# aoschu/esn-ofdm-mimo

Hardware: AMD Instinct MI355X
Metric: OFDM symbols/s through the ESN detector (4x8 TDL-B, N=128, N_res=512; train+predict+detect) (higher is better)
Workload: dtype f16 operands / f32 accumulate

## Files before the change

### esn_ofdm_mimo_amd/csrc/esn_solve.hip

```cpp
#include <stdlib.h>
#include <type_traits>
#include "esn_common.h"
#include "esn_launch.h"

namespace esn {

struct SolveParams {
    const double* E; const double* D;
    const float* E32;
    int n_groups, T, transient, cols, n_out;
    const double* t_scale; const double* t_shift;
    double* W_out; int* status;
    double* work; size_t work_stride;
    int m, n, wide;
    int skip;
    int part_ok;
    int vec;
    int dma;
    unsigned long long* stamps;
    const double* ridge; int n_ridge;
};

__device__ __forceinline__ bool ridge_rejects(const SolveParams& sp, int slot) {
    const double lam = sp.ridge[slot];
// ... 128 lines not shown
            double* z = R + (size_t)o * m;
            for (int j = 0; j < n; ++j) {
                const double* cj = M + (size_t)j * m;
                double acc = 0.0;
                for (int k = lane; k < j; k += 64) acc = fma(cj[k], z[k], acc);
                acc = wave_sum(acc);
                if (lane == 0) {
                    double d = rdiag[j];
                    z[j] = (fabs(d) > tol) ? (z[j] - acc) / d : 0.0;
                }
                __builtin_amdgcn_s_waitcnt(0);
                __builtin_amdgcn_wave_barrier();
            }
            for (int j = n - 1; j >= 0; --j) {
                const double* cj = M + (size_t)j * m;
                const double b = beta[j];
                if (b == 0.0) continue;
                double dot = 0.0;
                for (int i = j + lane; i < m; i += 64) dot = fma(cj[i], z[i], dot);
                dot = wave_sum(dot) * b;
                for (int i = j + lane; i < m; i += 64) z[i] = fma(-dot, cj[i], z[i]);
                __builtin_amdgcn_s_waitcnt(0);
                __builtin_amdgcn_wave_barrier();
            }
            double* wo = sp.W_out + ((size_t)slot * nrhs + o) * cols;
            for (int i = lane; i < cols; i += 64) wo[i] = z[i];
        }
    } else {
        for (int o = wv; o < nrhs; o += nwv) {
            double* c = M + (size_t)(n + o) * m;
            for (int j = n - 1; j >= 0; --j) {
                double acc = 0.0;
                for (int k = j + 1 + lane; k < n; k += 64) acc = fma(M[(size_t)k * m + j], c[k], acc);
                acc = wave_sum(acc);
                if (lane == 0) {
                    double d = rdiag[j];
                    c[j] = (fabs(d) > tol) ? (c[j] - acc) / d : 0.0;
                }
                __builtin_amdgcn_s_waitcnt(0);
                __builtin_amdgcn_wave_barrier();
            }
            double* wo = sp.W_out + ((size_t)slot * nrhs + o) * cols;
            for (int i = lane; i < n; i += 64) wo[i] = c[i];
        }
    }
}

size_t solve_work_doubles(int rows, int cols, int n_out) {
    const bool wide = rows < cols;
    const size_t m = wide ? cols : rows, n = wide ? rows : cols;
    size_t d = (n + (wide ? 0 : n_out)) * m + (size_t)n_out * m + 2 * n;
    return (d + 1) & ~(size_t)1;
}

size_t solve_ridge_work_doubles(int rows, int cols, int n_out) {
    const bool wide = rows < cols;
    const size_t m = (size_t)rows + cols, n = wide ? rows : cols;
    size_t d = (n + (wide ? 0 : n_out)) * m + (size_t)n_out * m + 2 * n;
    return (d + 1) & ~(size_t)1;
}

int launch_readout_solve(const double* E, const double* D, int n_groups, int T, int transient,
                         int cols, int n_out, const double* t_scale, const double* t_shift,
                         double* W_out, int* status, void* workspace, hipStream_t stream,
                         const double* ridge, int n_ridge) {
    SolveParams sp;
    const int rows = T - transient;
    sp.ridge = ridge; sp.n_ridge = n_ridge;
    sp.E = E; sp.E32 = nullptr; sp.D = D; sp.n_groups = n_groups; sp.T = T; sp.transient = transient;
    sp.cols = cols; sp.n_out = n_out; sp.t_scale = t_scale; sp.t_shift = t_shift;
    sp.W_out = W_out; sp.status = status;
    sp.work = reinterpret_cast<double*>(workspace);
    sp.work_stride = ridge ? solve_ridge_work_doubles(rows, cols, n_out) : solve_work_doubles(rows, cols, n_out);
    sp.wide = rows < cols;
    sp.m = sp.wide ? cols : rows;
    sp.n = sp.wide ? rows : cols;
    if (ridge) hipLaunchKernelGGL(readout_qr_kernel<true>, dim3(n_groups * n_ridge), dim3(1024), 0, stream, sp);
    else hipLaunchKernelGGL(readout_qr_kernel<false>, dim3(n_groups), dim3(1024), 0, stream, sp);
    return (int)hipGetLastError();
}

}

namespace esn {

constexpr int CH_NP = 128;
constexpr int CH_NT = 512;
constexpr int CH_NW = CH_NT / 64;
constexpr int CH_TILES = 36;
constexpr int CH_KC = 32;
constexpr int CH_AS_LD = CH_NP + 16;
constexpr int CH_RHS = 8;
constexpr size_t CH_LDS = sizeof(double) * ((size_t)CH_TILES * 256 + (size_t)CH_NP * CH_RHS);
static_assert(2 * CH_KC * CH_AS_LD <= CH_TILES * 256, "E staging aliases the Gram tiles");

typedef double f64x4 __attribute__((ext_vector_type(4)));

constexpr int CH_RING = 4;
constexpr int CH_RBUF = CH_KC * CH_NP * 4;
constexpr int CH_WRING = 3;
constexpr int CH_WSEG = 8192;
constexpr int CH_WROWS = 4;
static_assert(CH_RING * CH_RBUF <= CH_TILES * 256 * 8, "Gram ring aliases the Gram tiles");
static_assert(CH_WRING * 3 * CH_WSEG <= CH_TILES * 256 * 8, "W_out ring aliases the Gram tiles");

__device__ __forceinline__ __amdgpu_buffer_rsrc_t ch_rsrc(const void* ptr, int bytes) {
    const uint64_t a = (uint64_t)reinterpret_cast<uintptr_t>(ptr);
    const uint32_t lo = __builtin_amdgcn_readfirstlane((uint32_t)a);
    const uint32_t hi = __builtin_amdgcn_readfirstlane((uint32_t)(a >> 32));
    return __builtin_amdgcn_make_buffer_rsrc(reinterpret_cast<char*>((uintptr_t)(((uint64_t)hi << 32) | lo)), 0,
                                             __builtin_amdgcn_readfirstlane(bytes), 0x00020000);
}
__device__ __forceinline__ void ch_dma16(__amdgpu_buffer_rsrc_t rs, char* dst, int voff) {
    __builtin_amdgcn_raw_ptr_buffer_load_lds(rs, (__attribute__((address_space(3))) void*)dst, 16, voff, 0, 0, 0);
}
constexpr int CH_OOR = 0x7ffffff0;
__device__ __forceinline__ void ch_wait_dma(int pending) {
    switch (pending) {
        case 4: asm volatile("s_waitcnt vmcnt(4) lgkmcnt(0)" ::: "memory"); break;
        case 3: asm volatile("s_waitcnt vmcnt(3) lgkmcnt(0)" ::: "memory"); break;
        case 2: asm volatile("s_waitcnt vmcnt(2) lgkmcnt(0)" ::: "memory"); break;
        default: asm volatile("s_waitcnt vmcnt(0) lgkmcnt(0)" ::: "memory"); break;
    }
}

__device__ __forceinline__ void ch_wrow(const char* e, const double* al, float (&a)[4], double (&b)[8]) {
    typedef float f32x4 __attribute__((ext_vector_type(4)));
    typedef double f64x2 __attribute__((ext_vector_type(2)));
    const uint32_t ea = (uint32_t)(uintptr_t)(const __attribute__((address_space(3))) char*)e;
    const uint32_t ba = (uint32_t)(uintptr_t)(const __attribute__((address_space(3))) double*)al;
    f32x4 ev;
    f64x2 b0, b1, b2, b3;
    asm volatile("ds_read_b128 %0, %5\n\tds_read_b128 %1, %6\n\tds_read_b128 %2, %6 offset:16\n\t"
                 "ds_read_b128 %3, %6 offset:32\n\tds_read_b128 %4, %6 offset:48\n\ts_waitcnt lgkmcnt(0)"
                 : "=v"(ev), "=v"(b0), "=v"(b1), "=v"(b2), "=v"(b3) : "v"(ea), "v"(ba) : "memory");
    a[0] = ev.x; a[1] = ev.y; a[2] = ev.z; a[3] = ev.w;
    b[0] = b0.x; b[1] = b0.y; b[2] = b1.x; b[3] = b1.y; b[4] = b2.x; b[5] = b2.y; b[6] = b3.x; b[7] = b3.y;
}

__device__ __forceinline__ int ch_tile(int ti, int tj) { return (ti * (ti + 1) / 2 + tj) * 256; }
__device__ __forceinline__ int ch_el(int r, int c) { return r * 16 + (c ^ (r & ~1)); }

__device__ __forceinline__ void ch_load4(const float* p, float (&v)[4]) {
    const float4 x = *reinterpret_cast<const float4*>(p);
    v[0] = x.x; v[1] = x.y; v[2] = x.z; v[3] = x.w;
}
__device__ __forceinline__ void ch_load4(const double* p, double (&v)[4]) {
    const double2 x = *reinterpret_cast<const double2*>(p), y = *reinterpret_cast<const double2*>(p + 2);
    v[0] = x.x; v[1] = x.y; v[2] = y.x; v[3] = y.y;
}
__device__ __forceinline__ const float* ch_src(const SolveParams& sp, float*) { return sp.E32; }
__device__ __forceinline__ const double* ch_src(const SolveParams& sp, double*) { return sp.E; }

__device__ __forceinline__ double ch_bcast(double x, int src) {
    const uint64_t u = __builtin_bit_cast(uint64_t, x);
    const uint32_t lo = __builtin_amdgcn_readlane((uint32_t)u, src);
    const uint32_t hi = __builtin_amdgcn_readlane((uint32_t)(u >> 32), src);
    return __builtin_bit_cast(double, ((uint64_t)hi << 32) | lo);
}

__device__ __forceinline__ int ch_factor_diag(double* D, int j0, int n, double piv_tol, int lane) {
    const int r = lane & 15;
    double a[16], x[16];
#pragma unroll
    for (int c = 0; c < 16; ++c) a[c] = D[ch_el(r, c)];
    double my_invd = 1.0;
    unsigned rejected = 0, dropped = 0;
#pragma unroll
    for (int j = 0; j < 16; ++j) {
        const double v = ch_bcast(a[j], j);
        const bool live = j0 + j < n;
        const bool ok = live && v > piv_tol;
        if (live && !ok) rejected |= 1u << j;
        if (!ok) dropped |= 1u << j;
        const double d = ok ? sqrt(v) : 1.0, inv_d = ok ? 1.0 / d : 0.0;
        if (r == j) my_invd = ok ? inv_d : 1.0;
        a[j] = (r == j) ? d : ((r > j) ? a[j] * inv_d : 0.0);
#pragma unroll
        for (int k = j + 1; k < 16; ++k) {
            const double lkj = ch_bcast(a[j], k);
            if (r >= k) a[k] = fma(-a[j], lkj, a[k]);
        }
    }
#pragma unroll
    for (int i = 0; i < 16; ++i) {
        double sacc = (i == r) ? 1.0 : 0.0;
#pragma unroll
        for (int k = 0; k < i; ++k) sacc = fma(-ch_bcast(a[k], i), x[k], sacc);
        const double idi = ch_bcast(my_invd, i);
        x[i] = (i >= r && !((dropped >> i) & 1u)) ? sacc * idi : 0.0;
    }
    if (lane < 16) {
#pragma unroll
        for (int i = 0; i < 16; ++i) D[ch_el(i, r)] = x[i];
    }
    return rejected ? 1 : 0;
}

template <typename TE, bool wide, bool RG>
__global__ __launch_bounds__(CH_NT) __attribute__((amdgpu_waves_per_eu(4))) void readout_chol_kernel(SolveParams sp) {
    extern __shared__ __attribute__((aligned(16))) char chol_smem[];
    double* Gs = reinterpret_cast<double*>(chol_smem);
    double* As = Gs;
    double* Bs = Gs + CH_TILES * 256;
    const int slot = blockIdx.x, tid = threadIdx.x;
    const int g = RG ? slot / sp.n_ridge : slot;
    if constexpr (RG) {
        if (ridge_rejects(sp, slot)) return;
    }
    const int lane = tid & 63, wv = __builtin_amdgcn_readfirstlane(tid >> 6);
    const int lr = lane & 15, lq = lane >> 4;
    const int rows = sp.T - sp.transient, cols = sp.cols, nrhs = sp.n_out;
    const int n = wide ? rows : cols;
    const int m = wide ? cols : rows;
    const int ntile = (n + 15) / 16;
    const TE* A = ch_src(sp, (TE*)nullptr) + ((size_t)g * sp.T + sp.transient) * cols;
    const double* Dg = sp.D + ((size_t)g * sp.T + sp.transient) * nrhs;

    int g_ti[5], g_tj[5];
    const int g_cnt = wv < 4 ? 5 : 4;
#pragma unroll
    for (int q = 0; q < 5; ++q) {
        const int t = wv + CH_NW * q < CH_TILES ? wv + CH_NW * q : 0;
        int ti = 0;
        while ((ti + 1) * (ti + 2) / 2 <= t) ++ti;
        g_ti[q] = ti;
        g_tj[q] = t - ti * (ti + 1) / 2;
    }
    f64x4 acc[5];
#pragma unroll
    for (int q = 0; q < 5; ++q) acc[q] = f64x4{0.0, 0.0, 0.0, 0.0};
    double atb[2] = {0.0, 0.0};
    auto run_of = [&](int p, int& i, int& kk) {
        const int e = tid + CH_NT * p;
        if (wide) { i = (e & 15) + 16 * ((e >> 7) & 7); kk = 4 * ((e >> 4) & 7); }
        else      { kk = e >> 5; i = 4 * (e & 31); }
    };
    TE stg[2][4];
    auto fetch = [&](int k0) {
#pragma unroll
        for (int p = 0; p < 2; ++p) {
            int i, kk;
            run_of(p, i, kk);
            const int k = k0 + kk;
            int nv = wide ? (i < n ? m - k : 0) : (k < m ? n - i : 0);
            nv = nv < 0 ? 0 : (nv > 4 ? 4 : nv);
            const TE* src = A + (wide ? (size_t)i * cols + k : (size_t)k * cols + i);
            if (nv == 4 && sp.vec) {
                ch_load4(src, stg[p]);
            } else {
#pragma unroll
                for (int j = 0; j < 4; ++j) stg[p][j] = j < nv ? src[j] : (TE)0;
            }
        }
    };
    auto commit = [&](double* dst) {
#pragma unroll
        for (int p = 0; p < 2; ++p) {
            int i, kk;
            run_of(p, i, kk);
#pragma unroll
            for (int j = 0; j < 4; ++j) {
                if (wide) dst[(kk + j) * CH_AS_LD + i] = (double)stg[p][j];
                else      dst[kk * CH_AS_LD + i + j] = (double)stg[p][j];
            }
        }
    };
    double* Abuf[2] = {As, As + CH_KC * CH_AS_LD};
    const int m_run = (sp.skip & 1) ? CH_KC : m;
    constexpr bool can_dma = wide && sizeof(TE) == 4;
    const bool dma = can_dma && sp.dma && sp.vec;
#ifdef ESN_STAMPS
    unsigned long long st_acc[8] = {0, 0, 0, 0, 0, 0, 0, 0}, st_ph[4] = {0, 0, 0, 0};
    ESN_STAMP(st_k0);
#endif
    if constexpr (can_dma) {
        if (dma) {
            char* ring = chol_smem;
            const __amdgpu_buffer_rsrc_t ers = ch_rsrc(A, n * cols * 4);
            const int kq = lane >> 3;
            int roff[2];
#pragma unroll
            for (int j = 0; j < 2; ++j) roff[j] = ((16 * wv + 8 * j + (lane & 7)) * cols + 4 * kq) * 4;
            const int nch = (m_run + CH_KC - 1) / CH_KC;
            auto issue = [&](int c, int b) {
                const int k0 = c * CH_KC;
                const bool ok = k0 + 4 * kq < m;
#pragma unroll
                for (int j = 0; j < 2; ++j)
                    ch_dma16(ers, ring + b * CH_RBUF + (2 * wv + j) * 1024, ok ? roff[j] + 4 * k0 : CH_OOR);
            };
#pragma unroll
            for (int c = 0; c < CH_RING - 1; ++c)
                if (c < nch) issue(c, c);
            const int lbase = 1024 * (lr >> 3) + 16 * (lr & 7) + 4 * lq;
            for (int c = 0, b = 0; c < nch; ++c, b = (b + 1 == CH_RING ? 0 : b + 1)) {
#ifdef ESN_STAMPS
                ESN_STAMP(s0);
#endif
                const int later = nch - 1 - c < CH_RING - 2 ? nch - 1 - c : CH_RING - 2;
                ch_wait_dma(2 * later);
#ifdef ESN_STAMPS
                ESN_STAMP(s1);
#endif
                __builtin_amdgcn_s_barrier();
                if (c + CH_RING - 1 < nch) issue(c + CH_RING - 1, b == 0 ? CH_RING - 1 : b - 1);
                const char* buf = ring + b * CH_RBUF + lbase;
                const float* pa[5];
                const float* pb[5];
#pragma unroll
                for (int q = 0; q < 5; ++q) {
                    pa[q] = reinterpret_cast<const float*>(buf + 2048 * g_ti[q]);
                    pb[q] = reinterpret_cast<const float*>(buf + 2048 * g_tj[q]);
                }
#ifdef ESN_STAMPS
                ESN_STAMP(s2);
                {
                    float x = pa[0][0];
                    asm volatile("" :: "v"(x));
                }
                ESN_STAMP(s3);
#endif
                auto step = [&](int s, auto cnt) {
#pragma unroll
                    for (int q = 0; q < decltype(cnt)::value; ++q)
                        acc[q] = __builtin_amdgcn_mfma_f64_16x16x4f64((double)pa[q][32 * s], (double)pb[q][32 * s], acc[q], 0, 0, 0);
                };
                const int kmax = (m - c * CH_KC < CH_KC) ? m - c * CH_KC : CH_KC;
                if (kmax == CH_KC && g_cnt == 5) {
#pragma unroll
                    for (int s = 0; s < CH_KC / 4; ++s) step(s, std::integral_constant<int, 5>());
                } else if (kmax == CH_KC) {
#pragma unroll
                    for (int s = 0; s < CH_KC / 4; ++s) step(s, std::integral_constant<int, 4>());
                } else if (g_cnt == 5) {
                    for (int s = 0; s < kmax / 4; ++s) step(s, std::integral_constant<int, 5>());
                } else {
                    for (int s = 0; s < kmax / 4; ++s) step(s, std::integral_constant<int, 4>());
                }
#ifdef ESN_STAMPS
                ESN_STAMP(s4);
                st_acc[0] += s1 - s0; st_acc[1] += s2 - s1; st_acc[2] += s3 - s2; st_acc[3] += s4 - s3;
#endif
            }
            __syncthreads();
        }
    }
    for (int k0 = 0, cur = 0; k0 < (dma ? 0 : m_run); k0 += CH_KC, cur ^= 1) {
        if (k0 == 0) {
            fetch(0);
            commit(Abuf[0]);
            __syncthreads();
        }
#ifdef ESN_STAMPS
        ESN_STAMP(s0);
#endif
        if (k0 + CH_KC < m_run) fetch(k0 + CH_KC);
        const double* Ac = Abuf[cur];
        const int kmax = (m - k0 < CH_KC) ? m - k0 : CH_KC;
        const double* slab0 = Ac + lq * CH_AS_LD + lr;
        for (int k4 = 0; k4 < kmax; k4 += 4) {
            const double* slab = slab0 + k4 * CH_AS_LD;
#pragma unroll
            for (int q = 0; q < 5; ++q)
                if (q < g_cnt)
                    acc[q] = __builtin_amdgcn_mfma_f64_16x16x4f64(slab[g_ti[q] * 16], slab[g_tj[q] * 16], acc[q], 0, 0, 0);
        }
        if constexpr (!wide) {
#pragma unroll
            for (int p = 0; p < 2; ++p) {
                const int e = tid + CH_NT * p, o = e / CH_NP, i = e % CH_NP;
                if (o < nrhs) {
                    const double sc = sp.t_scale ? sp.t_scale[(size_t)g * nrhs + o] : 1.0;
                    const double sh = sp.t_shift ? sp.t_shift[(size_t)g * nrhs + o] : 0.0;
                    for (int kk = 0; kk < kmax; ++kk)
                        atb[p] = fma(Ac[kk * CH_AS_LD + i], Dg[(size_t)(k0 + kk) * nrhs + o] * sc + sh, atb[p]);
                }
            }
        }
#ifdef ESN_STAMPS
        ESN_STAMP(s1);
#endif
        if (k0 + CH_KC < m_run) commit(Abuf[cur ^ 1]);
#ifdef ESN_STAMPS
        ESN_STAMP(s2);
#endif
        __syncthreads();
#ifdef ESN_STAMPS
        ESN_STAMP(s3);
        st_acc[3] += s1 - s0; st_acc[0] += s2 - s1; st_acc[1] += s3 - s2;
#endif
    }
#ifdef ESN_STAMPS
    ESN_STAMP(st_k1);
#endif

#pragma unroll
    for (int q = 0; q < 5; ++q)
        if (q < g_cnt) {
            double* T = Gs + ch_tile(g_ti[q], g_tj[q]);
#pragma unroll
            for (int i = 0; i < 4; ++i) T[ch_el(4 * i + lq, lr)] = acc[q][i];
        }
#pragma unroll
    for (int p = 0; p < 2; ++p) {
        const int e = tid + CH_NT * p;
        if (wide) {
            const int i = e / CH_RHS, o = e % CH_RHS;
            double v = 0.0;
            if (i < n && o < nrhs) {
                const double sc = sp.t_scale ? sp.t_scale[(size_t)g * nrhs + o] : 1.0;
                const double sh = sp.t_shift ? sp.t_shift[(size_t)g * nrhs + o] : 0.0;
                v = Dg[(size_t)i * nrhs + o] * sc + sh;
            }
            Bs[e] = v;
        } else {
            const int o = e / CH_NP, i = e % CH_NP;
            Bs[i * CH_RHS + o] = (o < nrhs && i < n) ? atb[p] : 0.0;
        }
    }
    __syncthreads();
    if constexpr (RG) {
        const double lam = sp.ridge[slot];
        for (int i = tid; i < n; i += CH_NT) Gs[ch_tile(i >> 4, i >> 4) + ch_el(i & 15, i & 15)] += lam;
        __syncthreads();
    }

    int bad = 0;
    const int nblk = (sp.skip & 2) ? 1 : ntile;
    double piv_tol = 0.0;
    if (wv == 0) {
        double dmax = 0.0;
        for (int i = lane; i < n; i += 64) dmax = fmax(dmax, Gs[ch_tile(i >> 4, i >> 4) + ch_el(i & 15, i & 15)]);
#pragma unroll
        for (int off = 32; off > 0; off >>= 1) dmax = fmax(dmax, __shfl_xor(dmax, off));
        piv_tol = dmax * 1e-14;
    }
    for (int kb = -1; kb < nblk; ++kb) {
        if (kb >= 0) {
            const int rt = kb + 1 + wv;
            if (rt < ntile) {
                const double* Li = Gs + ch_tile(kb, kb);

                double* T = Gs + ch_tile(rt, kb);
                f64x4 c = {0.0, 0.0, 0.0, 0.0};
#pragma unroll
                for (int k0 = 0; k0 < 16; k0 += 4)
                    c = __builtin_amdgcn_mfma_f64_16x16x4f64(T[ch_el(lr, k0 + lq)], Li[ch_el(lr, k0 + lq)], c, 0, 0, 0);
#pragma unroll
                for (int i = 0; i < 4; ++i) T[ch_el(4 * i + lq, lr)] = c[i];
            }
        }
        if (kb >= 0) {
            __syncthreads();
            const int mt = ntile - kb - 1, cnt = mt * (mt + 1) / 2;
            for (int t = wv; t < cnt; t += (wv == 0 ? cnt : CH_NW - 1)) {
                int di = 0;
                while ((di + 1) * (di + 2) / 2 <= t) ++di;
                const int ti = kb + 1 + di, tj = kb + 1 + t - di * (di + 1) / 2;
                double* C = Gs + ch_tile(ti, tj);
                const double* La = Gs + ch_tile(ti, kb);
                const double* Lb = Gs + ch_tile(tj, kb);
                f64x4 c;
#pragma unroll
                for (int i = 0; i < 4; ++i) c[i] = C[ch_el(4 * i + lq, lr)];
#pragma unroll
                for (int k0 = 0; k0 < 16; k0 += 4)
                    c = __builtin_amdgcn_mfma_f64_16x16x4f64(-La[ch_el(lr, k0 + lq)], Lb[ch_el(lr, k0 + lq)], c, 0, 0, 0);
#pragma unroll
                for (int i = 0; i < 4; ++i) C[ch_el(4 * i + lq, lr)] = c[i];
            }
        }
        if (wv == 0 && kb + 1 < nblk) bad |= ch_factor_diag(Gs + ch_tile(kb + 1, kb + 1), 16 * (kb + 1), n, piv_tol, lane);
        __syncthreads();
    }

#ifdef ESN_STAMPS
    ESN_STAMP(st_k2);
#endif
    if (!(sp.skip & 4)) {
        const bool bl = lr < CH_RHS;
        f64x4 keep = {0.0, 0.0, 0.0, 0.0};
        int keep_t = -1;
        auto rhs_tile = [&](int I) -> f64x4 {
            f64x4 v;
#pragma unroll
            for (int i = 0; i < 4; ++i) v[i] = bl ? Bs[(16 * I + 4 * i + lq) * CH_RHS + lr] : 0.0;
            return v;
        };
        auto put_tile = [&](int I, const f64x4& v) {
            if (bl) {
#pragma unroll
                for (int i = 0; i < 4; ++i) Bs[(16 * I + 4 * i + lq) * CH_RHS + lr] = v[i];
            }
        };
        auto flush = [&]() {
            if (wv == CH_NW - 1 && keep_t >= 0) put_tile(keep_t, keep);
            keep_t = -1;
        };
        for (int I = 0; I < ntile; ++I) {
            flush();
            const int J = I + 1 + wv;
            const bool upd = J < ntile;
            if (upd || wv == CH_NW - 1) {
                const double* Li = Gs + ch_tile(I, I);
                const f64x4 b = rhs_tile(I);
                f64x4 z = {0.0, 0.0, 0.0, 0.0};
#pragma unroll
                for (int s = 0; s < 4; ++s)
                    z = __builtin_amdgcn_mfma_f64_16x16x4f64(Li[ch_el(lr, 4 * s + lq)], b[s], z, 0, 0, 0);
                if (upd) {
                    const double* L = Gs + ch_tile(J, I);
                    f64x4 c = rhs_tile(J);
#pragma unroll
                    for (int s = 0; s < 4; ++s)
                        c = __builtin_amdgcn_mfma_f64_16x16x4f64(-L[ch_el(lr, 4 * s + lq)], z[s], c, 0, 0, 0);
                    put_tile(J, c);
                } else {
                    keep = z;
                    keep_t = I;
                }
            }
            __syncthreads();
        }
        flush();
        __syncthreads();
        for (int I = ntile - 1; I >= 0; --I) {
            flush();
            const int J = wv;
            const bool upd = J < I;
            if (upd || wv == CH_NW - 1) {
                const double* Li = Gs + ch_tile(I, I);
                const f64x4 zi = rhs_tile(I);
                f64x4 x = {0.0, 0.0, 0.0, 0.0};
#pragma unroll
                for (int s = 0; s < 4; ++s)
                    x = __builtin_amdgcn_mfma_f64_16x16x4f64(Li[ch_el(4 * s + lq, lr)], zi[s], x, 0, 0, 0);
                if (upd) {
                    const double* L = Gs + ch_tile(I, J);
                    f64x4 c = rhs_tile(J);
#pragma unroll
                    for (int s = 0; s < 4; ++s)
                        c = __builtin_amdgcn_mfma_f64_16x16x4f64(-L[ch_el(4 * s + lq, lr)], x[s], c, 0, 0, 0);
                    put_tile(J, c);
                } else {
                    keep = x;
                    keep_t = I;
                }
            }
            __syncthreads();
        }
        flush();
        __syncthreads();
    }

#ifdef ESN_STAMPS
    ESN_STAMP(st_k3);
#endif
    if constexpr (wide) {
        constexpr int CPT = 16 / sizeof(TE);
        const int nunit = cols / CPT;
        int parts = nunit > 0 ? CH_NT / nunit : 0;
        parts = parts > 3 ? 3 : parts;
        if (sp.vec && cols % CPT == 0 && parts > 0 && (parts - 1) * CH_RHS * cols <= CH_TILES * 256 && !(sp.skip & 8)) {
            double* part = Gs;
            const int pt = tid / nunit, un = tid - pt * nunit;
            double w[CPT][CH_RHS];
#pragma unroll
            for (int c = 0; c < CPT; ++c)
#pragma unroll
                for (int o = 0; o < CH_RHS; ++o) w[c][o] = 0.0;
            const int per = (n + parts - 1) / parts;
            int rw = CH_WSEG / (cols * 4);
            rw = rw > CH_WROWS ? CH_WROWS : rw;
            bool wdma = false;
            if constexpr (can_dma) {
              wdma = dma && rw > 0;
              if (wdma) {
                char* ring = chol_smem;
                const __amdgpu_buffer_rsrc_t ers = ch_rsrc(A, n * cols * 4);
                const int rowb = cols * 4;
                const int nch = (per + rw - 1) / rw;
                auto issue = [&](int c, int b) {
#pragma unroll
                    for (int j = 0; j < 3; ++j) {
                        const int r0 = j * per + c * rw;
                        int nr = (j < parts) ? ((j + 1) * per < n ? (j + 1) * per : n) - r0 : 0;
                        nr = nr < 0 ? 0 : (nr > rw ? rw : nr);
                        const int off = 1024 * wv + 16 * lane;
                        ch_dma16(ers, ring + (b * 3 + j) * CH_WSEG + 1024 * wv, off < nr * rowb ? r0 * rowb + off : CH_OOR);
                    }
                };
#pragma unroll
                for (int c = 0; c < CH_WRING - 1; ++c)
                    if (c < nch) issue(c, c);
                const int i0 = pt * per, i1 = (i0 + per < n) ? i0 + per : n;
                for (int c = 0, b = 0; c < nch; ++c, b = (b + 1 == CH_WRING ? 0 : b + 1)) {
#ifdef ESN_STAMPS
                    ESN_STAMP(s0);
#endif
                    ch_wait_dma(nch - 1 - c < CH_WRING - 2 ? 3 * (nch - 1 - c) : 3 * (CH_WRING - 2));
#ifdef ESN_STAMPS
                    ESN_STAMP(s1);
#endif
                    __builtin_amdgcn_s_barrier();
                    if (c + CH_WRING - 1 < nch) issue(c + CH_WRING - 1, b == 0 ? CH_WRING - 1 : b - 1);
#ifdef ESN_STAMPS
                    ESN_STAMP(s2);
#endif
                    if (pt < parts) {
                        const char* seg = ring + (b * 3 + pt) * CH_WSEG + CPT * sizeof(TE) * un;
                        const int ib = i0 + c * rw;
                        const int nr = ((ib + rw < i1) ? ib + rw : i1) - ib;
#pragma unroll
                        for (int rr = 0; rr < CH_WROWS; ++rr) {
                            if (rr >= nr) break;
                            const int i = ib + rr;
                            float a[4];
                            double al[CH_RHS];
                            ch_wrow(seg + rr * rowb, Bs + i * CH_RHS, a, al);
#pragma unroll
                            for (int o = 0; o < CH_RHS; ++o)
                                if (o < nrhs) {
#pragma unroll
                                    for (int cc = 0; cc < CPT; ++cc) w[cc][o] = fma((double)a[cc], al[o], w[cc][o]);
                                }
                        }
                    }
#ifdef ESN_STAMPS
                    ESN_STAMP(s3);
                    st_acc[4] += s1 - s0; st_acc[5] += s2 - s1; st_acc[6] += s3 - s2;
#endif
                }
                __syncthreads();
                if (pt > 0 && pt < parts) {
#pragma unroll
                    for (int o = 0; o < CH_RHS; ++o)
                        if (o < nrhs) {
#pragma unroll
                            for (int c = 0; c < CPT; ++c) part[((pt - 1) * CH_RHS + o) * cols + CPT * un + c] = w[c][o];
                        }
                }
              }
            }
            if (!wdma && pt < parts) {
                const int i0 = pt * per, i1 = (i0 + per < n) ? i0 + per : n;
                const TE* ac = A + (size_t)CPT * un;
#pragma unroll 4
                for (int i = i0; i < i1; ++i) {
                    TE a[CPT];
                    if constexpr (CPT == 4) {
                        ch_load4(ac + (size_t)i * cols, a);
                    } else {
                        const double2 ad = *reinterpret_cast<const double2*>(ac + (size_t)i * cols);
                        a[0] = ad.x; a[1] = ad.y;
                    }
#pragma unroll
                    for (int o = 0; o < CH_RHS; ++o)
                        if (o < nrhs) {
                            const double al = Bs[i * CH_RHS + o];
#pragma unroll
                            for (int c = 0; c < CPT; ++c) w[c][o] = fma((double)a[c], al, w[c][o]);
                        }
                }
                if (pt > 0) {
#pragma unroll
                    for (int o = 0; o < CH_RHS; ++o)
                        if (o < nrhs) {
#pragma unroll
                            for (int c = 0; c < CPT; ++c) part[((pt - 1) * CH_RHS + o) * cols + CPT * un + c] = w[c][o];
                        }
                }
            }
            __syncthreads();
            if (pt == 0) {
#pragma unroll
                for (int o = 0; o < CH_RHS; ++o)
                    if (o < nrhs) {
#pragma unroll
                        for (int c = 0; c < CPT; ++c) {
                            double v = w[c][o];
                            for (int q = 1; q < parts; ++q) v += part[((q - 1) * CH_RHS + o) * cols + CPT * un + c];
                            sp.W_out[((size_t)slot * nrhs + o) * cols + CPT * un + c] = v;
                        }
                    }
            }
        } else {
            for (int c = tid; c < ((sp.skip & 8) ? 0 : cols); c += CH_NT) {
                double w[CH_RHS];
#pragma unroll
                for (int o = 0; o < CH_RHS; ++o) w[o] = 0.0;
#pragma unroll 8
                for (int i = 0; i < n; ++i) {
                    const double a = (double)A[(size_t)i * cols + c];
#pragma unroll
                    for (int o = 0; o < CH_RHS; ++o)
                        if (o < nrhs) w[o] = fma(a, Bs[i * CH_RHS + o], w[o]);
                }
#pragma unroll
                for (int o = 0; o < CH_RHS; ++o)
                    if (o < nrhs) sp.W_out[((size_t)slot * nrhs + o) * cols + c] = w[o];
            }
        }
    } else {
        for (int e = tid; e < nrhs * cols; e += CH_NT) {
            const int o = e / cols, c = e % cols;
            sp.W_out[((size_t)slot * nrhs + o) * cols + c] = Bs[c * CH_RHS + o];
        }
    }
    if (tid == 0) sp.status[slot] = bad;
#ifdef ESN_STAMPS
    ESN_STAMP(st_k4);
    if (sp.stamps && slot == 0 && lane == 0) {
        for (int i = 0; i < 7; ++i) sp.stamps[wv * 8 + i] = st_acc[i];
        sp.stamps[(8 + wv) * 8 + 0] = st_k1 - st_k0;
        sp.stamps[(8 + wv) * 8 + 1] = st_k2 - st_k1;
        sp.stamps[(8 + wv) * 8 + 2] = st_k3 - st_k2;
        sp.stamps[(8 + wv) * 8 + 3] = st_k4 - st_k3;
        sp.stamps[(8 + wv) * 8 + 4] = st_k4 - st_k0;
    }
#endif
}

int launch_readout_chol(const double* E, const float* E32, const double* D, int n_groups, int T, int transient,
                        int cols, int n_out, const double* t_scale, const double* t_shift,
                        double* W_out, int* status, hipStream_t stream, const double* ridge, int n_ridge) {
    SolveParams sp;
    sp.E32 = E32;
    sp.ridge = ridge; sp.n_ridge = n_ridge;
    const int rows = T - transient;
    const int n = rows < cols ? rows : cols;
    if (n > CH_NP || n_out > CH_RHS) return -1;
    sp.E = E; sp.D = D; sp.n_groups = n_groups; sp.T = T; sp.transient = transient;
    sp.cols = cols; sp.n_out = n_out; sp.t_scale = t_scale; sp.t_shift = t_shift;
    sp.W_out = W_out; sp.status = status; sp.work = nullptr; sp.work_stride = 0;
    sp.wide = rows < cols; sp.m = sp.wide ? cols : rows; sp.n = n;
    sp.skip = knobs().chol_skip;
    sp.dma = knobs().chol_dma;
    sp.part_ok = 0;
#ifdef ESN_STAMPS
    sp.stamps = stamp_buffer();
#else
    sp.stamps = nullptr;
#endif
    const uintptr_t base = E32 ? (uintptr_t)E32 : (uintptr_t)E;
    sp.vec = (base % 16 == 0) && (cols % (E32 ? 4 : 2) == 0);
    void (*fn)(SolveParams);
    if (ridge)
        fn = E32 ? (sp.wide ? readout_chol_kernel<float, true, true> : readout_chol_kernel<float, false, true>)
                 : (sp.wide ? readout_chol_kernel<double, true, true> : readout_chol_kernel<double, false, true>);
    else
        fn = E32 ? (sp.wide ? readout_chol_kernel<float, true, false> : readout_chol_kernel<float, false, false>)
                 : (sp.wide ? readout_chol_kernel<double, true, false> : readout_chol_kernel<double, false, false>);
    hipError_t e = hipFuncSetAttribute(reinterpret_cast<const void*>(fn), hipFuncAttributeMaxDynamicSharedMemorySize,
                                       (int)CH_LDS);
    if (e != hipSuccess) return (int)e;
    hipLaunchKernelGGL(fn, dim3(ridge ? n_groups * n_ridge : n_groups), dim3(CH_NT), CH_LDS, stream, sp);
    return (int)hipGetLastError();
}

}

namespace esn {

constexpr int CB_NMAX = 512;
constexpr int CB_KC = 8;
constexpr int CB_PLD = 17;
constexpr int CB_NT = 512;
constexpr int CB_NW = CB_NT / 64;
constexpr int CB_EPT = CB_NMAX * CB_KC / CB_NT;
constexpr int CB_TPW = 16;

size_t chol_big_work_doubles(int n) {
    const size_t np = (size_t)round_up(n, 16);
    return np * np;
}

template <bool RG>
__global__ __launch_bounds__(CB_NT) void readout_chol_big_kernel(SolveParams sp) {
    extern __shared__ __attribute__((aligned(16))) char cb_smem[];
    typedef double f64x4 __attribute__((ext_vector_type(4)));
    __shared__ int sh_bad;
    __shared__ double sh_invd[CB_NMAX];
    __shared__ double sh_linv[16][17];
    __shared__ double sh_red[CB_NW];
    const int slot = blockIdx.x, tid = threadIdx.x;
    const int g = RG ? slot / sp.n_ridge : slot;
    if constexpr (RG) {
        if (ridge_rejects(sp, slot)) return;
    }
    const int lane = tid & 63, wv = tid >> 6;
    const int wvu = __builtin_amdgcn_readfirstlane(wv);
    const int rows = sp.T - sp.transient, cols = sp.cols, nrhs = sp.n_out;
    const bool wide = rows < cols;
    const int n = wide ? rows : cols;
    const int m = wide ? cols : rows;
    const int np = round_up(n, 16), ntile = np / 16;
    const int ld = np;
    double* Gw = sp.work + (size_t)slot * sp.work_stride;
    const size_t a_off = ((size_t)g * sp.T + sp.transient) * cols;
    const double* A = sp.E ? sp.E + a_off : nullptr;
    const float* A32 = sp.E32 ? sp.E32 + a_off : nullptr;
    const double* Dg = sp.D + ((size_t)g * sp.T + sp.transient) * nrhs;
    const int lr = lane & 15, lq = lane >> 4;
    if (tid == 0) sh_bad = 0;

    {
        const int AS_LD = np + 4;
        double* Abuf[2] = {reinterpret_cast<double*>(cb_smem), reinterpret_cast<double*>(cb_smem) + (size_t)CB_KC * AS_LD};
        const int ept = (np * CB_KC + CB_NT - 1) / CB_NT;
        double stg[CB_EPT];
        auto fetch = [&](int k0) {
#pragma unroll
            for (int q = 0; q < CB_EPT; ++q) {
                const int e = tid + CB_NT * q;
                int kk, i;
                if (wide) { i = e / CB_KC; kk = e % CB_KC; } else { kk = e / np; i = e % np; }
                const int k = k0 + kk;
                const size_t ai_ = wide ? (size_t)i * cols + k : (size_t)k * cols + i;
                stg[q] = (q < ept && e < np * CB_KC && i < n && k < m) ? (A32 ? (double)A32[ai_] : A[ai_]) : 0.0;
            }
        };
        auto commit = [&](double* dst) {
#pragma unroll
            for (int q = 0; q < CB_EPT; ++q) {
                const int e = tid + CB_NT * q;
                if (q < ept && e < np * CB_KC) {
                    int kk, i;
                    if (wide) { i = e / CB_KC; kk = e % CB_KC; } else { kk = e / np; i = e % np; }
                    dst[kk * AS_LD + i] = stg[q];
                }
            }
        };
        const int fr_off = lq * AS_LD + lr;
        const int n_pass = (ntile + 3) / 4;
        for (int jb = 0; jb < n_pass; ++jb) {
            const int tj0 = 4 * jb, tj1 = (tj0 + 4 < ntile) ? tj0 + 4 : ntile;
            int cnt = 0;
            for (int tj = tj0; tj < tj1; ++tj) cnt += ntile - tj;
            int my_ti[CB_TPW], my_tj[CB_TPW];
#pragma unroll
            for (int q = 0; q < CB_TPW; ++q) {
                int t = wvu + CB_NW * q, tj = tj0;
                bool ok = t < cnt;
                while (ok && t >= ntile - tj) { t -= ntile - tj; ++tj; }
                my_tj[q] = ok ? tj : -1;
                my_ti[q] = ok ? tj + t : 0;
            }
            f64x4 acc[CB_TPW];
#pragma unroll
            for (int q = 0; q < CB_TPW; ++q) acc[q] = f64x4{0.0, 0.0, 0.0, 0.0};
            fetch(0);
            commit(Abuf[0]);
            __syncthreads();
            int cur = 0;
            for (int k0 = 0; k0 < m; k0 += CB_KC) {
                const bool more = k0 + CB_KC < m;
                if (more) fetch(k0 + CB_KC);
                const double* Ac = Abuf[cur];
#pragma unroll
                for (int k4 = 0; k4 < CB_KC; k4 += 4) {
                    const double* slab = Ac + k4 * AS_LD + fr_off;
#pragma unroll
                    for (int q = 0; q < CB_TPW; ++q)
                        if (my_tj[q] >= 0)
                            acc[q] = __builtin_amdgcn_mfma_f64_16x16x4f64(slab[my_ti[q] * 16], slab[my_tj[q] * 16], acc[q], 0, 0, 0);
                }
                if (more) commit(Abuf[cur ^ 1]);
                __syncthreads();
                cur ^= 1;
            }
#pragma unroll
            for (int q = 0; q < CB_TPW; ++q)
                if (my_tj[q] >= 0) {
#pragma unroll
                    for (int i = 0; i < 4; ++i)
                        Gw[(size_t)(my_tj[q] * 16 + lr) * ld + my_ti[q] * 16 + 4 * i + lq] = acc[q][i];
                }
            __syncthreads();
        }
        double* Bs = reinterpret_cast<double*>(cb_smem);
        __syncthreads();
        for (int e = tid; e < nrhs * np; e += CB_NT) {
            const int o = e / np, i = e % np;
            double v = 0.0;
            if (wide && i < n) {
                const double sc = sp.t_scale ? sp.t_scale[(size_t)g * nrhs + o] : 1.0;
                const double sh = sp.t_shift ? sp.t_shift[(size_t)g * nrhs + o] : 0.0;
                v = Dg[(size_t)i * nrhs + o] * sc + sh;
            }
            if (wide) Bs[e] = v;
        }
        if (!wide) {
            for (int e = tid; e < nrhs * np; e += CB_NT) {
                const int o = e / np, i = e % np;
                double acc_b = 0.0;
                if (i < n) {
                    const double sc = sp.t_scale ? sp.t_scale[(size_t)g * nrhs + o] : 1.0;
                    const double sh = sp.t_shift ? sp.t_shift[(size_t)g * nrhs + o] : 0.0;
#pragma unroll 8
                    for (int k = 0; k < m; ++k) {
                        const double a = A32 ? (double)A32[(size_t)k * cols + i] : A[(size_t)k * cols + i];
                        acc_b = fma(a, Dg[(size_t)k * nrhs + o] * sc + sh, acc_b);
                    }
                }
                Bs[e] = acc_b;
            }
        }
        if constexpr (RG) {
            const double lam = sp.ridge[slot];
            for (int i = tid; i < n; i += CB_NT) Gw[(size_t)i * ld + i] += lam;
        }
    }
    __threadfence_block();
    __syncthreads();
    double* Bs = reinterpret_cast<double*>(cb_smem);
    double* P = Bs + (size_t)8 * CB_NMAX;
    double dmax = 0.0;
    for (int i = tid; i < n; i += CB_NT) dmax = fmax(dmax, Gw[(size_t)i * ld + i]);
#pragma unroll
    for (int off = 32; off > 0; off >>= 1) dmax = fmax(dmax, __shfl_down(dmax, off));
    if (lane == 0) sh_red[wv] = dmax;
    __syncthreads();
    double piv_tol = 0.0;
    for (int w = 0; w < CB_NW; ++w) piv_tol = fmax(piv_tol, sh_red[w]);
    piv_tol *= 1e-14;

    auto bcast = [](double x, int src) -> double {
        const uint64_t u = __builtin_bit_cast(uint64_t, x);
        const uint32_t lo = __builtin_amdgcn_readlane((uint32_t)u, src);
        const uint32_t hi = __builtin_amdgcn_readlane((uint32_t)(u >> 32), src);
        return __builtin_bit_cast(double, ((uint64_t)hi << 32) | lo);
    };
    for (int j = 0; j < ntile; ++j) {
        const int j0 = 16 * j;
        for (int rt = j + wvu; rt < ntile; rt += CB_NW) {
            f64x4 c;
#pragma unroll
            for (int i = 0; i < 4; ++i) c[i] = Gw[(size_t)(j0 + lr) * ld + rt * 16 + 4 * i + lq];
            const double* la = Gw + (size_t)lq * ld + rt * 16 + lr;
            const double* lb = Gw + (size_t)lq * ld + j0 + lr;
#pragma unroll 4
            for (int k = 0; k < j0; k += 4)
                c = __builtin_amdgcn_mfma_f64_16x16x4f64(-la[(size_t)k * ld], lb[(size_t)k * ld], c, 0, 0, 0);
#pragma unroll
            for (int i = 0; i < 4; ++i) P[(rt * 16 + 4 * i + lq) * CB_PLD + lr] = c[i];
        }
        __syncthreads();
        if (wv == 0) {
            const int r = lane & 15;
            double a[16], x[16];
#pragma unroll
            for (int c = 0; c < 16; ++c) a[c] = P[(j0 + r) * CB_PLD + c];
            double my_invd = 1.0;
            unsigned rejected = 0;
#pragma unroll
            for (int jj = 0; jj < 16; ++jj) {
                const double v = bcast(a[jj], jj);
                const bool live = j0 + jj < n;
                const bool ok = live && v > piv_tol;
                if (live && !ok) rejected |= 1u << jj;
                const double d = ok ? sqrt(v) : 1.0, inv_d = ok ? 1.0 / d : 0.0;
                if (r == jj) my_invd = ok ? inv_d : 1.0;
                a[jj] = (r == jj) ? d : ((r > jj) ? a[jj] * inv_d : 0.0);
#pragma unroll
                for (int k = jj + 1; k < 16; ++k) {
                    const double lkj = bcast(a[jj], k);
                    if (r >= k) a[k] = fma(-a[jj], lkj, a[k]);
                }
            }
            if (lane < 16) {
#pragma unroll
                for (int c = 0; c < 16; ++c) P[(j0 + r) * CB_PLD + c] = a[c];
                sh_invd[j0 + r] = my_invd;
            }
            if (rejected && lane == 0) sh_bad = 1;
#pragma unroll
            for (int i = 0; i < 16; ++i) {
                double sacc = (i == r) ? 1.0 : 0.0;
#pragma unroll
                for (int k = 0; k < i; ++k) sacc = fma(-bcast(a[k], i), x[k], sacc);
                const double idi = bcast(my_invd, i);
                x[i] = (i >= r && !((rejected >> i) & 1u)) ? sacc * idi : 0.0;
            }
            if (lane < 16) {
#pragma unroll
                for (int i = 0; i < 16; ++i) sh_linv[i][r] = x[i];
            }
        }
        __syncthreads();
        for (int rt = j + 1 + wvu; rt < ntile; rt += CB_NW) {
            f64x4 c = {0.0, 0.0, 0.0, 0.0};
#pragma unroll
            for (int k0 = 0; k0 < 16; k0 += 4)
                c = __builtin_amdgcn_mfma_f64_16x16x4f64(P[(rt * 16 + lr) * CB_PLD + k0 + lq], sh_linv[lr][k0 + lq], c, 0, 0, 0);
            __builtin_amdgcn_wave_barrier();
#pragma unroll
            for (int i = 0; i < 4; ++i) P[(rt * 16 + 4 * i + lq) * CB_PLD + lr] = c[i];
        }
        __syncthreads();
        for (int e = tid; e < (np - j0) * 16; e += CB_NT) {
            const int c = e / (np - j0), rr = j0 + e % (np - j0);
            Gw[(size_t)(j0 + c) * ld + rr] = P[rr * CB_PLD + c];
        }
        __threadfence_block();
        __syncthreads();
    }

    if (wv < nrhs) {
        double* xb = Bs + (size_t)wv * np;
        constexpr int NS = CB_NMAX / 64;
        const int ns = (np + 63) / 64;
        double b[NS], l[NS], lnext[NS];
#pragma unroll
        for (int s2 = 0; s2 < NS; ++s2) b[s2] = (s2 < ns && lane + 64 * s2 < np) ? xb[lane + 64 * s2] : 0.0;
        auto load_col = [&](double (&dst)[NS], int jc) {
#pragma unroll
            for (int s2 = 0; s2 < NS; ++s2) {
                const int i = lane + 64 * s2;
                dst[s2] = (s2 < ns && jc >= 0 && jc < n && i < n) ? Gw[(size_t)jc * ld + i] : 0.0;
            }
        };
        auto pick = [&](const double (&v)[NS], int jc) -> double {
            double own = 0.0;
#pragma unroll
            for (int s2 = 0; s2 < NS; ++s2) own = ((jc >> 6) == s2) ? v[s2] : own;
            return __shfl(own, jc & 63);
        };
        load_col(l, 0);
        for (int jc = 0; jc < n; ++jc) {
            load_col(lnext, jc + 1);
            const double zj = pick(b, jc) * sh_invd[jc];
#pragma unroll
            for (int s2 = 0; s2 < NS; ++s2) {
                const int i = lane + 64 * s2;
                b[s2] = (i == jc) ? zj : ((i > jc) ? fma(-l[s2], zj, b[s2]) : b[s2]);
            }
#pragma unroll
            for (int s2 = 0; s2 < NS; ++s2) l[s2] = lnext[s2];
        }
        load_col(l, n - 1);
        for (int jc = n - 1; jc >= 0; --jc) {
            load_col(lnext, jc - 1);
            double part = 0.0;
#pragma unroll
            for (int s2 = 0; s2 < NS; ++s2) {
                const int i = lane + 64 * s2;
                part = (i > jc && i < n) ? fma(l[s2], b[s2], part) : part;
            }
            part = wave_sum(part);
            const double xj = (pick(b, jc) - part) * sh_invd[jc];
#pragma unroll
            for (int s2 = 0; s2 < NS; ++s2) b[s2] = (lane + 64 * s2 == jc) ? xj : b[s2];
#pragma unroll
            for (int s2 = 0; s2 < NS; ++s2) l[s2] = lnext[s2];
        }
#pragma unroll
        for (int s2 = 0; s2 < NS; ++s2)
            if (s2 < ns && lane + 64 * s2 < np) xb[lane + 64 * s2] = b[s2];
    }
    __syncthreads();

    if (wide) {
        double* part = P;
        if (sp.part_ok) {
            const int cpt = A32 ? 4 : 2, nunit = cols / cpt;
            int parts = CB_NT / nunit;
            if (parts > 3) parts = 3;
            const int pt = tid / nunit, un = tid - pt * nunit;
            if (pt < parts) {
                const int per = (n + parts - 1) / parts;
                const int i0 = pt * per, i1 = (i0 + per < n) ? i0 + per : n;
                double w[4][8];
#pragma unroll
                for (int c = 0; c < 4; ++c)
#pragma unroll
                    for (int o = 0; o < 8; ++o) w[c][o] = 0.0;
                const size_t ac = (size_t)cpt * un;
#pragma unroll 4
                for (int i = i0; i < i1; ++i) {
                    double a[4];
                    if (A32) {
                        const float4 af = *reinterpret_cast<const float4*>(A32 + ac + (size_t)i * cols);
                        a[0] = (double)af.x; a[1] = (double)af.y; a[2] = (double)af.z; a[3] = (double)af.w;
                    } else {
                        const double2 ad = *reinterpret_cast<const double2*>(A + ac + (size_t)i * cols);
                        a[0] = ad.x; a[1] = ad.y; a[2] = 0.0; a[3] = 0.0;
                    }
#pragma unroll
                    for (int o = 0; o < 8; ++o)
                        if (o < nrhs) {
                            const double al = Bs[o * np + i];
#pragma unroll
                            for (int c = 0; c < 4; ++c)
                                if (c < cpt) w[c][o] = fma(a[c], al, w[c][o]);
                        }
                }
#pragma unroll
                for (int o = 0; o < 8; ++o)
                    if (o < nrhs) {
#pragma unroll
                        for (int c = 0; c < 4; ++c)
                            if (c < cpt) part[(pt * 8 + o) * cols + cpt * un + c] = w[c][o];
                    }
            }
            __syncthreads();
            for (int e = tid; e < nrhs * cols; e += CB_NT) {
                const int o = e / cols, c = e - o * cols;
                double v = part[o * cols + c];
                for (int q = 1; q < parts; ++q) v += part[(q * 8 + o) * cols + c];
                sp.W_out[((size_t)slot * nrhs + o) * cols + c] = v;
            }
        } else {
            for (int c = tid; c < cols; c += CB_NT) {
                double w[8];
#pragma unroll
                for (int o = 0; o < 8; ++o) w[o] = 0.0;
                for (int i = 0; i < n; ++i) {
                    const double a = A32 ? (double)A32[(size_t)i * cols + c] : A[(size_t)i * cols + c];
#pragma unroll
                    for (int o = 0; o < 8; ++o)
                        if (o < nrhs) w[o] = fma(a, Bs[o * np + i], w[o]);
                }
#pragma unroll
                for (int o = 0; o < 8; ++o)
                    if (o < nrhs) sp.W_out[((size_t)slot * nrhs + o) * cols + c] = w[o];
            }
        }
    } else {
        for (int e = tid; e < nrhs * cols; e += CB_NT) {
            const int o = e / cols, c = e % cols;
            sp.W_out[((size_t)slot * nrhs + o) * cols + c] = Bs[o * np + c];
        }
    }
    if (tid == 0) sp.status[slot] = sh_bad;
}

// ... 43 lines not shown
```

Before: 11.70 million.

## Rewrite 16x16 diagonal Cholesky block with DPP row-broadcast FMAs and fused inverse

Replaces the readlane-based scalar broadcasts in the 16x16 diagonal-tile Cholesky factor and triangular inverse with inline-asm DPP row_newbcast moves and v_fmac_f64_dpp. The inverse of L is now built column by column alongside the factorization rather than in a second forward-substitution pass. The point is to shorten the serial critical path that one wave runs between barriers in both Cholesky kernels. It relies on hand-written asm with s_nop hazard padding and changes the masking of dropped pivots, which could affect correctness or portability. It also adds per-phase timing stamps behind ESN_STAMPS.

```diff
diff --git a/esn_ofdm_mimo_amd/csrc/esn_solve.hip b/esn_ofdm_mimo_amd/csrc/esn_solve.hip
--- a/esn_ofdm_mimo_amd/csrc/esn_solve.hip
+++ b/esn_ofdm_mimo_amd/csrc/esn_solve.hip
@@ -304,44 +304,92 @@
 __device__ __forceinline__ const float* ch_src(const SolveParams& sp, float*) { return sp.E32; }
 __device__ __forceinline__ const double* ch_src(const SolveParams& sp, double*) { return sp.E; }
 
-__device__ __forceinline__ double ch_bcast(double x, int src) {
-    const uint64_t u = __builtin_bit_cast(uint64_t, x);
-    const uint32_t lo = __builtin_amdgcn_readlane((uint32_t)u, src);
-    const uint32_t hi = __builtin_amdgcn_readlane((uint32_t)(u >> 32), src);
-    return __builtin_bit_cast(double, ((uint64_t)hi << 32) | lo);
-}
-
-__device__ __forceinline__ int ch_factor_diag(double* D, int j0, int n, double piv_tol, int lane) {
-    const int r = lane & 15;
-    double a[16], x[16];
-#pragma unroll
-    for (int c = 0; c < 16; ++c) a[c] = D[ch_el(r, c)];
-    double my_invd = 1.0;
-    unsigned rejected = 0, dropped = 0;
-#pragma unroll
-    for (int j = 0; j < 16; ++j) {
-        const double v = ch_bcast(a[j], j);
+template <int SRC>
+__device__ __forceinline__ double ch_row_bcast(double x) {
+    double v;
+    asm("s_nop 4\n\tv_mov_b64_dpp %0, %1 row_newbcast:%c2 row_mask:0xf bank_mask:0xf" : "=v"(v) : "v"(x), "i"(SRC));
+    return v;
+}
+
+#define CH_DPP_FMAC(t) "v_fmac_f64_dpp %" #t ", -%[d], %[o] row_newbcast:%c[l" #t "] row_mask:0xf bank_mask:0xf\n\t"
+template <int L0, int N>
+__device__ __forceinline__ void ch_dpp_fmac(double* acc, double d, double o) {
+    static_assert(N == 8 || N == 4 || N == 2 || N == 1, "group sizes");
+    static_assert(L0 >= 0 && L0 + N <= 16, "lanes of one row");
+    if constexpr (N == 8) {
+        asm("s_nop 4\n\t" CH_DPP_FMAC(0) CH_DPP_FMAC(1) CH_DPP_FMAC(2) CH_DPP_FMAC(3)
+            CH_DPP_FMAC(4) CH_DPP_FMAC(5) CH_DPP_FMAC(6) CH_DPP_FMAC(7)
+            : "+v"(acc[0]), "+v"(acc[1]), "+v"(acc[2]), "+v"(acc[3]), "+v"(acc[4]), "+v"(acc[5]), "+v"(acc[6]), "+v"(acc[7])
+            : [d] "v"(d), [o] "v"(o), [l0] "i"(L0), [l1] "i"(L0 + 1), [l2] "i"(L0 + 2), [l3] "i"(L0 + 3),
+              [l4] "i"(L0 + 4), [l5] "i"(L0 + 5), [l6] "i"(L0 + 6), [l7] "i"(L0 + 7));
+    } else if constexpr (N == 4) {
+        asm("s_nop 4\n\t" CH_DPP_FMAC(0) CH_DPP_FMAC(1) CH_DPP_FMAC(2) CH_DPP_FMAC(3)
+            : "+v"(acc[0]), "+v"(acc[1]), "+v"(acc[2]), "+v"(acc[3])
+            : [d] "v"(d), [o] "v"(o), [l0] "i"(L0), [l1] "i"(L0 + 1), [l2] "i"(L0 + 2), [l3] "i"(L0 + 3));
+    } else if constexpr (N == 2) {
+        asm("s_nop 4\n\t" CH_DPP_FMAC(0) CH_DPP_FMAC(1)
+            : "+v"(acc[0]), "+v"(acc[1]) : [d] "v"(d), [o] "v"(o), [l0] "i"(L0), [l1] "i"(L0 + 1));
+    } else {
+        asm("s_nop 4\n\t" CH_DPP_FMAC(0) : "+v"(acc[0]) : [d] "v"(d), [o] "v"(o), [l0] "i"(L0));
+    }
+}
+#undef CH_DPP_FMAC
+template <int FROM>
+__device__ __forceinline__ void ch_dpp_fmac_from(double (&acc)[16], double d, double o) {
+    constexpr int cnt = 16 - FROM;
+    if constexpr (cnt & 8) ch_dpp_fmac<FROM, 8>(acc + FROM, d, o);
+    if constexpr (cnt & 4) ch_dpp_fmac<FROM + (cnt & 8), 4>(acc + FROM + (cnt & 8), d, o);
+    if constexpr (cnt & 2) ch_dpp_fmac<FROM + (cnt & 12), 2>(acc + FROM + (cnt & 12), d, o);
+    if constexpr (cnt & 1) ch_dpp_fmac<15, 1>(acc + 15, d, o);
+}
+
+template <bool DROP_PAD, bool FULL_L>
+__device__ __forceinline__ unsigned ch_diag_regs(double (&a)[16], double (&x)[16], double& my_invd, int j0, int n,
+                                                 double piv_tol, int r) {
+    my_invd = 1.0;
+    unsigned rejected = 0;
+#pragma unroll
+    for (int i = 0; i < 16; ++i) x[i] = (i == r) ? 1.0 : 0.0;
+    double v = ch_row_bcast<0>(a[0]);
+    auto column = [&](auto jc) {
+        constexpr int j = decltype(jc)::value;
         const bool live = j0 + j < n;
         const bool ok = live && v > piv_tol;
         if (live && !ok) rejected |= 1u << j;
-        if (!ok) dropped |= 1u << j;
-        const double d = ok ? sqrt(v) : 1.0, inv_d = ok ? 1.0 / d : 0.0;
-        if (r == j) my_invd = ok ? inv_d : 1.0;
-        a[j] = (r == j) ? d : ((r > j) ? a[j] * inv_d : 0.0);
-#pragma unroll
-        for (int k = j + 1; k < 16; ++k) {
-            const double lkj = ch_bcast(a[j], k);
-            if (r >= k) a[k] = fma(-a[j], lkj, a[k]);
-        }
-    }
-#pragma unroll
-    for (int i = 0; i < 16; ++i) {
-        double sacc = (i == r) ? 1.0 : 0.0;
-#pragma unroll
-        for (int k = 0; k < i; ++k) sacc = fma(-ch_bcast(a[k], i), x[k], sacc);
-        const double idi = ch_bcast(my_invd, i);
-        x[i] = (i >= r && !((dropped >> i) & 1u)) ? sacc * idi : 0.0;
-    }
+        const double d = sqrt(ok ? v : 1.0), inv_1 = 1.0 / d, inv_d = ok ? inv_1 : 0.0;
+        if constexpr (FULL_L) {
+            if (r == j) my_invd = inv_1;
+            a[j] = (r == j) ? d : ((r > j) ? a[j] * inv_d : 0.0);
+        } else {
+            a[j] *= inv_d;
+        }
+        if constexpr (j < 15) {
+            ch_dpp_fmac<j + 1, 1>(a + j + 1, a[j], a[j]);
+            v = ch_row_bcast<j + 1>(a[j + 1]);
+        }
+        if constexpr (j < 14) ch_dpp_fmac_from<j + 2>(a, a[j], a[j]);
+        const bool zero = DROP_PAD ? !ok : live && !ok;
+        x[j] = (j >= r && !zero) ? x[j] * inv_1 : 0.0;
+        if constexpr (j < 15) ch_dpp_fmac_from<j + 1>(x, a[j], x[j]);
+    };
+    column(std::integral_constant<int, 0>()); column(std::integral_constant<int, 1>());
+    column(std::integral_constant<int, 2>()); column(std::integral_constant<int, 3>());
+    column(std::integral_constant<int, 4>()); column(std::integral_constant<int, 5>());
+    column(std::integral_constant<int, 6>()); column(std::integral_constant<int, 7>());
+    column(std::integral_constant<int, 8>()); column(std::integral_constant<int, 9>());
+    column(std::integral_constant<int, 10>()); column(std::integral_constant<int, 11>());
+    column(std::integral_constant<int, 12>()); column(std::integral_constant<int, 13>());
+    column(std::integral_constant<int, 14>()); column(std::integral_constant<int, 15>());
+    return rejected;
+}
+
+__device__ __forceinline__ int ch_factor_diag(double* D, int j0, int n, double piv_tol, int lane) {
+    int r = lane & 15;
+    asm volatile("" : "+v"(r));
+    double a[16], x[16], my_invd;
+#pragma unroll
+    for (int c = 0; c < 16; ++c) a[c] = D[ch_el(r, c)];
+    const unsigned rejected = ch_diag_regs<true, false>(a, x, my_invd, j0, n, piv_tol, r);
     if (lane < 16) {
 #pragma unroll
         for (int i = 0; i < 16; ++i) D[ch_el(i, r)] = x[i];
@@ -589,6 +637,10 @@
         piv_tol = dmax * 1e-14;
     }
     for (int kb = -1; kb < nblk; ++kb) {
+#ifdef ESN_STAMPS
+        ESN_STAMP(f0);
+        unsigned long long f1 = f0, f2 = f0;
+#endif
         if (kb >= 0) {
             const int rt = kb + 1 + wv;
             if (rt < ntile) {
@@ -604,7 +656,13 @@
             }
         }
         if (kb >= 0) {
+#ifdef ESN_STAMPS
+            ESN_STAMP_SET(f1);
+#endif
             __syncthreads();
+#ifdef ESN_STAMPS
+            ESN_STAMP_SET(f2);
+#endif
             const int mt = ntile - kb - 1, cnt = mt * (mt + 1) / 2;
             for (int t = wv; t < cnt; t += (wv == 0 ? cnt : CH_NW - 1)) {
                 int di = 0;
@@ -623,8 +681,18 @@
                 for (int i = 0; i < 4; ++i) C[ch_el(4 * i + lq, lr)] = c[i];
             }
         }
+#ifdef ESN_STAMPS
+        ESN_STAMP(f3);
+#endif
         if (wv == 0 && kb + 1 < nblk) bad |= ch_factor_diag(Gs + ch_tile(kb + 1, kb + 1), 16 * (kb + 1), n, piv_tol, lane);
+#ifdef ESN_STAMPS
+        ESN_STAMP(f4);
+#endif
         __syncthreads();
+#ifdef ESN_STAMPS
+        ESN_STAMP(f5);
+        st_ph[0] += (f1 - f0) + (f3 - f2); st_ph[1] += (f2 - f1) + (f5 - f4); st_ph[2] += f4 - f3;
+#endif
     }
 
 #ifdef ESN_STAMPS
@@ -870,6 +938,7 @@
         sp.stamps[(8 + wv) * 8 + 2] = st_k3 - st_k2;
         sp.stamps[(8 + wv) * 8 + 3] = st_k4 - st_k3;
         sp.stamps[(8 + wv) * 8 + 4] = st_k4 - st_k0;
+        for (int i = 0; i < 3; ++i) sp.stamps[(8 + wv) * 8 + 5 + i] = st_ph[i];
     }
 #endif
 }
@@ -1078,12 +1147,6 @@
     for (int w = 0; w < CB_NW; ++w) piv_tol = fmax(piv_tol, sh_red[w]);
     piv_tol *= 1e-14;
 
-    auto bcast = [](double x, int src) -> double {
-        const uint64_t u = __builtin_bit_cast(uint64_t, x);
-        const uint32_t lo = __builtin_amdgcn_readlane((uint32_t)u, src);
-        const uint32_t hi = __builtin_amdgcn_readlane((uint32_t)(u >> 32), src);
-        return __builtin_bit_cast(double, ((uint64_t)hi << 32) | lo);
-    };
     for (int j = 0; j < ntile; ++j) {
         const int j0 = 16 * j;
         for (int rt = j + wvu; rt < ntile; rt += CB_NW) {
@@ -1101,40 +1164,16 @@
         __syncthreads();
         if (wv == 0) {
             const int r = lane & 15;
-            double a[16], x[16];
+            double a[16], x[16], my_invd;
 #pragma unroll
             for (int c = 0; c < 16; ++c) a[c] = P[(j0 + r) * CB_PLD + c];
-            double my_invd = 1.0;
-            unsigned rejected = 0;
-#pragma unroll
-            for (int jj = 0; jj < 16; ++jj) {
-                const double v = bcast(a[jj], jj);
-                const bool live = j0 + jj < n;
-                const bool ok = live && v > piv_tol;
-                if (live && !ok) rejected |= 1u << jj;
-                const double d = ok ? sqrt(v) : 1.0, inv_d = ok ? 1.0 / d : 0.0;
-                if (r == jj) my_invd = ok ? inv_d : 1.0;
-                a[jj] = (r == jj) ? d : ((r > jj) ? a[jj] * inv_d : 0.0);
-#pragma unroll
-                for (int k = jj + 1; k < 16; ++k) {
-                    const double lkj = bcast(a[jj], k);
-                    if (r >= k) a[k] = fma(-a[jj], lkj, a[k]);
-                }
-            }
+            const unsigned rejected = ch_diag_regs<false, true>(a, x, my_invd, j0, n, piv_tol, r);
             if (lane < 16) {
 #pragma unroll
                 for (int c = 0; c < 16; ++c) P[(j0 + r) * CB_PLD + c] = a[c];
                 sh_invd[j0 + r] = my_invd;
             }
             if (rejected && lane == 0) sh_bad = 1;
-#pragma unroll
-            for (int i = 0; i < 16; ++i) {
-                double sacc = (i == r) ? 1.0 : 0.0;
-#pragma unroll
-                for (int k = 0; k < i; ++k) sacc = fma(-bcast(a[k], i), x[k], sacc);
-                const double idi = bcast(my_invd, i);
-                x[i] = (i >= r && !((rejected >> i) & 1u)) ? sacc * idi : 0.0;
-            }
             if (lane < 16) {
 #pragma unroll
                 for (int i = 0; i < 16; ++i) sh_linv[i][r] = x[i];
```

Measured after the change: 11.84 million, median of 6. 1.01x the previous value.
